# OpenDriveLab/ThinkTwice

Measured on AMD Instinct MI355X. Metric: frames/sec forward (4-cam+LiDAR, thinktwice.py cfg), higher is better.
Workload: dtype bf16x3h; 1 GPU; forward_inference thinktwice.py cfg: 8 frames x (2 sweeps x 4 cams x 448x896 + 65536-pt LiDAR), ResNet50+PAFPN+DepthNet+UNet+LSS splat, LidarNet, fusion, 5-stage decoder; parallelism=replicas x1 (no data-path collective), launch=eager launches, 3 batches in flight on alternating streams, batches_in_flight=3

## Files before the change

### thinktwice_amd/csrc/lidar.hip

```cpp
#include <hipcub/hipcub.hpp>

#include "tt_common.h"

namespace tt {

constexpr unsigned long long kInvalidKey = ~0ull;

struct Dims3 { int z, y, x; };

__global__ void lidar_keys_kernel(const float* __restrict__ pts, int B, int Np, int nfeat, float x0, float y0,
                                  float z0, float vx, float vy, float vz, int gx, int gy, int gz, int zlimit,
                                  unsigned long long* __restrict__ keys, unsigned* __restrict__ vals) {
#pragma clang fp contract(off)
    const long long i = (long long)blockIdx.x * blockDim.x + threadIdx.x;
    if (i >= (long long)B * Np) return;
    const int b = (int)(i / Np);
    const float* p = pts + i * nfeat;
    const int cx = (int)floorf((p[0] - x0) / vx);
    const int cy = (int)floorf((p[1] - y0) / vy);
    const int cz = (int)floorf((p[2] - z0) / vz);
    const bool ok = cx >= 0 && cx < gx && cy >= 0 && cy < gy && cz >= 0 && cz < gz && cz < zlimit;
    keys[i] = ok ? ((((unsigned long long)b * gz + cz) * gy + cy) * gx + cx) : kInvalidKey;
    vals[i] = (unsigned)i;
}

__global__ void mark_heads_kernel(const unsigned long long* __restrict__ keys, long long n, int* __restrict__ flags,
                                  int* __restrict__ n_valid) {
    const long long i = (long long)blockIdx.x * blockDim.x + threadIdx.x;
    if (i >= n) return;
    const unsigned long long k = keys[i];
    const bool valid = k != kInvalidKey;
    flags[i] = (valid && (i == 0 || keys[i - 1] != k)) ? 1 : 0;
    if (valid && (i == n - 1 || keys[i + 1] == kInvalidKey)) *n_valid = (int)(i + 1);
}

__global__ void voxel_heads_kernel(const unsigned long long* __restrict__ keys, const int* __restrict__ flags,
                                   const int* __restrict__ scan, long long n, int gx, int gy, int gz,
                                   int* __restrict__ coords, int* __restrict__ first, int* __restrict__ num_voxels) {
    const long long i = (long long)blockIdx.x * blockDim.x + threadIdx.x;
    if (i >= n) return;
    if (flags[i]) {
        const int v = scan[i];
        unsigned long long k = keys[i];
        const int x = (int)(k % gx); k /= gx;
        const int y = (int)(k % gy); k /= gy;
        const int z = (int)(k % gz); k /= gz;
        coords[v * 4 + 0] = (int)k;
        coords[v * 4 + 1] = z;
        coords[v * 4 + 2] = y;
        coords[v * 4 + 3] = x;
        first[v] = (int)i;
    }
    if (i == n - 1) *num_voxels = scan[i] + flags[i];
}

__global__ void vfe_mean_kernel(const float* __restrict__ pts, const unsigned* __restrict__ vals,
                                const int* __restrict__ first, const int* __restrict__ num_voxels,
                                const int* __restrict__ n_valid, int nfeat, int max_points, long long max_rows,
                                float* __restrict__ feats) {
    const long long t = (long long)blockIdx.x * blockDim.x + threadIdx.x;
    const long long v = t / nfeat;
    const int f = (int)(t % nfeat);
    const int M = *num_voxels;
    if (v >= M || v >= max_rows) return;
    const int s = first[v];
    const int e = (v + 1 < M) ? first[v + 1] : *n_valid;
    const int cnt = min(e - s, max_points);
    float sum = 0.f;
    for (int j = 0; j < cnt; ++j) sum += pts[(long long)vals[s + j] * nfeat + f];
    feats[v * nfeat + f] = sum / (float)cnt;
}


__global__ void cap_head_points_kernel(const unsigned long long* __restrict__ keys, const int* __restrict__ flags,
                                       const int* __restrict__ scan_h, const unsigned* __restrict__ vals, long long n,
                                       int* __restrict__ head_pos, int* __restrict__ pt_flag, int* __restrict__ n_heads) {
    const long long i = (long long)blockIdx.x * blockDim.x + threadIdx.x;
    if (i >= n) return;
    if (flags[i]) {
        head_pos[scan_h[i]] = (int)i;
        pt_flag[vals[i]] = 1;
    }
    if (i == n - 1) *n_heads = scan_h[i] + flags[i];
}

__global__ void cap_keep_kernel(const unsigned long long* __restrict__ keys, const int* __restrict__ flags,
                                const unsigned* __restrict__ vals, const int* __restrict__ scan_p, long long n, int Np, int gx,
                                int gy, int gz, int zlimit, int max_voxels, int* __restrict__ keep) {
    const long long i = (long long)blockIdx.x * blockDim.x + threadIdx.x;
    if (i >= n) return;
    int k = 0;
    if (flags[i]) {
        unsigned long long key = keys[i];
        key /= gx; key /= gy;
        const int z = (int)(key % gz);
        const long long p = vals[i];
        const long long b = p / Np;
        const int rank = scan_p[p] - scan_p[b * Np];
        k = (rank < max_voxels && z < zlimit) ? 1 : 0;
    }
    keep[i] = k;
}

__global__ void cap_emit_kernel(const unsigned long long* __restrict__ keys, const int* __restrict__ keep,
                                const int* __restrict__ scan_k, const int* __restrict__ scan_h,
                                const int* __restrict__ head_pos, const int* __restrict__ n_heads,
                                const int* __restrict__ n_valid, long long n, int gx, int gy, int gz, int* __restrict__ coords,
                                int* __restrict__ first, int* __restrict__ last, int* __restrict__ num_voxels) {
    const long long i = (long long)blockIdx.x * blockDim.x + threadIdx.x;
    if (i >= n) return;
    if (keep[i]) {
        const int v = scan_k[i], h = scan_h[i];
        unsigned long long k = keys[i];
        const int x = (int)(k % gx); k /= gx;
        const int y = (int)(k % gy); k /= gy;
        const int z = (int)(k % gz); k /= gz;
        coords[v * 4 + 0] = (int)k;
        coords[v * 4 + 1] = z;
        coords[v * 4 + 2] = y;
        coords[v * 4 + 3] = x;
        first[v] = (int)i;
        last[v] = (h + 1 < *n_heads) ? head_pos[h + 1] : *n_valid;
    }
    if (i == n - 1) *num_voxels = scan_k[i] + keep[i];
}

__global__ void vfe_mean_capped_kernel(const float* __restrict__ pts, const unsigned* __restrict__ vals,
                                       const int* __restrict__ first, const int* __restrict__ last,
                                       const int* __restrict__ num_voxels, int nfeat, int max_points, long long max_rows,
                                       float* __restrict__ feats) {
    const long long t = (long long)blockIdx.x * blockDim.x + threadIdx.x;
    const long long v = t / nfeat;
    const int f = (int)(t % nfeat);
    if (v >= *num_voxels || v >= max_rows) return;
    const int s = first[v];
    const int cnt = min(last[v] - s, max_points);
    float sum = 0.f;
    for (int j = 0; j < cnt; ++j) sum += pts[(long long)vals[s + j] * nfeat + f];
    feats[v * nfeat + f] = sum / (float)cnt;
}

struct ConvGeom { int kz, ky, kx, sz, sy, sx, pz, py, px; };

__device__ __forceinline__ long long lin_cell(int b, int z, int y, int x, Dims3 d) {
    return (((long long)b * d.z + z) * d.y + y) * d.x + x;
}

__global__ void volume_scatter_kernel(const int* __restrict__ coords, const int* __restrict__ num_rows,
                                      long long max_rows, Dims3 d, int* __restrict__ vol) {
    const long long i = (long long)blockIdx.x * blockDim.x + threadIdx.x;
    if (i >= *num_rows || i >= max_rows) return;
    vol[lin_cell(coords[i * 4], coords[i * 4 + 1], coords[i * 4 + 2], coords[i * 4 + 3], d)] = (int)i;
}

__global__ void mark_outputs_kernel(const int* __restrict__ in_coords, const int* __restrict__ in_rows,
                                    long long max_in, ConvGeom g, Dims3 od, int* __restrict__ flags) {
    const int KV = g.kz * g.ky * g.kx;
    const long long t = (long long)blockIdx.x * blockDim.x + threadIdx.x;
    const long long i = t / KV;
    const int k = (int)(t % KV);
    if (i >= *in_rows || i >= max_in) return;
    const int kz = k / (g.ky * g.kx), ky = (k / g.kx) % g.ky, kx = k % g.kx;
    const int nz = in_coords[i * 4 + 1] + g.pz - kz;
    const int ny = in_coords[i * 4 + 2] + g.py - ky;
    const int nx = in_coords[i * 4 + 3] + g.px - kx;
    if (nz < 0 || ny < 0 || nx < 0 || nz % g.sz || ny % g.sy || nx % g.sx) return;
    const int oz = nz / g.sz, oy = ny / g.sy, ox = nx / g.sx;
    if (oz >= od.z || oy >= od.y || ox >= od.x) return;
    flags[lin_cell(in_coords[i * 4], oz, oy, ox, od)] = 1;
}

__global__ void compact_outputs_kernel(const int* __restrict__ flags, const int* __restrict__ scan, long long cells,
                                       Dims3 od, long long max_out, int* __restrict__ vol,
                                       int* __restrict__ out_coords, int* __restrict__ out_rows) {
    const long long c = (long long)blockIdx.x * blockDim.x + threadIdx.x;
    if (c >= cells) return;
    const int f = flags[c];
    const int row = scan[c];
    int v = -1;
    if (f && row < max_out) {
        v = row;
        long long r = c;
        const int x = (int)(r % od.x); r /= od.x;
        const int y = (int)(r % od.y); r /= od.y;
        const int z = (int)(r % od.z); r /= od.z;
        out_coords[(long long)row * 4 + 0] = (int)r;
        out_coords[(long long)row * 4 + 1] = z;
        out_coords[(long long)row * 4 + 2] = y;
        out_coords[(long long)row * 4 + 3] = x;
    }
    vol[c] = v;
    if (c == cells - 1) {
        const long long n = (long long)row + f;
        *out_rows = (int)(n < max_out ? n : max_out);
    }
}

__global__ void rulebook_kernel(const int* __restrict__ out_coords, const int* __restrict__ out_rows, long long max_out,
                                ConvGeom g, Dims3 id, const int* __restrict__ vol, int* __restrict__ nbr) {
    const int KV = g.kz * g.ky * g.kx;
    const long long t = (long long)blockIdx.x * blockDim.x + threadIdx.x;
    const long long o = t / KV;
    const int k = (int)(t % KV);
    if (o >= *out_rows || o >= max_out) return;
    const int kz = k / (g.ky * g.kx), ky = (k / g.kx) % g.ky, kx = k % g.kx;
    const int z = out_coords[o * 4 + 1] * g.sz - g.pz + kz;
    const int y = out_coords[o * 4 + 2] * g.sy - g.py + ky;
    const int x = out_coords[o * 4 + 3] * g.sx - g.px + kx;
    int r = -1;
    if (z >= 0 && z < id.z && y >= 0 && y < id.y && x >= 0 && x < id.x)
        r = vol[lin_cell(out_coords[o * 4], z, y, x, id)];
    nbr[o * KV + k] = r;
}

__global__ void sp_row_masks_kernel(const int* __restrict__ nbr, const int* __restrict__ rows_n, long long max_rows, int KV,
                                    unsigned* __restrict__ keys, unsigned* __restrict__ vals,
                                    unsigned long long* __restrict__ pairs) {
    const long long o = (long long)blockIdx.x * blockDim.x + threadIdx.x;
    unsigned cnt = 0;
    if (o < max_rows) {
        unsigned m = 0xFFFFFFFFu;
        if (o < *rows_n) {
            m = 0;
            for (int t = 0; t < KV; ++t) m |= (nbr[o * KV + t] >= 0 ? 1u : 0u) << t;
            cnt = __popc(m);
        }
        keys[o] = m;
        vals[o] = (unsigned)o;
    }
    if (pairs) {
#pragma unroll
        for (int off = 32; off > 0; off >>= 1) cnt += __shfl_xor(cnt, off);
        if ((threadIdx.x & 63) == 0 && cnt) atomicAdd(pairs, (unsigned long long)cnt);
    }
}

template <typename T>
__global__ void sp_to_dense_kernel(const T* __restrict__ f, const int* __restrict__ coords,
                                   const int* __restrict__ rows_n, long long max_rows, int C, Dims3 d,
                                   T* __restrict__ dense) {
    const long long t = (long long)blockIdx.x * blockDim.x + threadIdx.x;
    const long long r = t / C;
    const int c = (int)(t % C);
    if (r >= *rows_n || r >= max_rows) return;
    const int b = coords[r * 4], z = coords[r * 4 + 1], y = coords[r * 4 + 2], x = coords[r * 4 + 3];
    dense[(((long long)b * d.y + y) * d.x + x) * ((long long)C * d.z) + (long long)c * d.z + z] = f[r * C + c];
}

}

using namespace tt;

static size_t align256(size_t v) { return (v + 255) / 256 * 256; }

extern "C" long long tt_lidar_voxelize_workspace_bytes(long long num_points_total) {
    size_t sort_bytes = 0, scan_bytes = 0;
    const int n = (int)num_points_total;
    (void)hipcub::DeviceRadixSort::SortPairs(nullptr, sort_bytes, (unsigned long long*)nullptr,
                                       (unsigned long long*)nullptr, (unsigned*)nullptr, (unsigned*)nullptr, n);
    (void)hipcub::DeviceScan::ExclusiveSum(nullptr, scan_bytes, (int*)nullptr, (int*)nullptr, n);
    size_t tot = 0;
    tot += 2 * align256(sizeof(unsigned long long) * n);
    tot += 2 * align256(sizeof(unsigned) * n);
    tot += 2 * align256(sizeof(int) * n);
    tot += align256(sizeof(int) * (n + 1));
    tot += align256(sizeof(int) * 4);
    tot += align256(sort_bytes > scan_bytes ? sort_bytes : scan_bytes);
    return (long long)tot;
}

extern "C" int tt_lidar_voxelize(const float* points, int B, int Np, int nfeat, const float* pc_range_lo,
                                 const float* voxel_size, const int* grid_xyz, int z_limit, int max_points,
                                 void* workspace, long long workspace_bytes, float* voxel_feats, int* coords,
                                 int* num_voxels, void* stream) {
    TT_REQUIRE(points && pc_range_lo && voxel_size && grid_xyz && workspace && voxel_feats && coords && num_voxels,
               "tt_lidar_voxelize: null");
    const long long n = (long long)B * Np;
    TT_REQUIRE(n > 0 && n < (1ll << 30), "tt_lidar_voxelize: bad point count");
    TT_REQUIRE(workspace_bytes >= tt_lidar_voxelize_workspace_bytes(n), "tt_lidar_voxelize: workspace too small");
    hipStream_t st = (hipStream_t)stream;
    char* w = (char*)workspace;
    auto take = [&](size_t bytes) { char* p = w; w += align256(bytes); return p; };
    auto* keys_in = (unsigned long long*)take(sizeof(unsigned long long) * n);
    auto* keys_out = (unsigned long long*)take(sizeof(unsigned long long) * n);
    auto* vals_in = (unsigned*)take(sizeof(unsigned) * n);
    auto* vals_out = (unsigned*)take(sizeof(unsigned) * n);
    auto* flags = (int*)take(sizeof(int) * n);
    auto* scan = (int*)take(sizeof(int) * n);
    auto* first = (int*)take(sizeof(int) * (n + 1));
    auto* n_valid = (int*)take(sizeof(int) * 4);
    void* tmp = w;
    size_t tmp_bytes = (size_t)(workspace_bytes - (w - (char*)workspace));
    (void)hipMemsetAsync(n_valid, 0, sizeof(int), st);
    (void)hipMemsetAsync(num_voxels, 0, sizeof(int), st);
    const unsigned blocks = (unsigned)div_up(n, 256);
    hipLaunchKernelGGL(lidar_keys_kernel, dim3(blocks), dim3(256), 0, st, points, B, Np, nfeat, pc_range_lo[0],
                       pc_range_lo[1], pc_range_lo[2], voxel_size[0], voxel_size[1], voxel_size[2], grid_xyz[0],
                       grid_xyz[1], grid_xyz[2], z_limit, keys_in, vals_in);
    size_t sb = tmp_bytes;
    if (hipcub::DeviceRadixSort::SortPairs(tmp, sb, keys_in, keys_out, vals_in, vals_out, (int)n, 0, 64, st) !=
        hipSuccess) {
        set_error("tt_lidar_voxelize: radix sort failed");
        return -2;
    }
    hipLaunchKernelGGL(mark_heads_kernel, dim3(blocks), dim3(256), 0, st, keys_out, n, flags, n_valid);
    sb = tmp_bytes;
    if (hipcub::DeviceScan::ExclusiveSum(tmp, sb, flags, scan, (int)n, st) != hipSuccess) {
        set_error("tt_lidar_voxelize: scan failed");
        return -2;
    }
    hipLaunchKernelGGL(voxel_heads_kernel, dim3(blocks), dim3(256), 0, st, keys_out, flags, scan, n, grid_xyz[0],
                       grid_xyz[1], grid_xyz[2], coords, first, num_voxels);
    hipLaunchKernelGGL(vfe_mean_kernel, dim3((unsigned)div_up(n * nfeat, 256)), dim3(256), 0, st, points, vals_out,
                       first, num_voxels, n_valid, nfeat, max_points, n, voxel_feats);
    return check_launch("tt_lidar_voxelize");
}


extern "C" long long tt_lidar_voxelize_capped_workspace_bytes(long long num_points_total) {
    const long long n = num_points_total;
    return tt_lidar_voxelize_workspace_bytes(n) + (long long)(8 * align256(sizeof(int) * (n + 1)));
}

extern "C" int tt_lidar_voxelize_capped(const float* points, int B, int Np, int nfeat, const float* pc_range_lo,
                                        const float* voxel_size, const int* grid_xyz, int z_limit, int max_points,
                                        int max_voxels, void* workspace, long long workspace_bytes, float* voxel_feats,
                                        int* coords, int* num_voxels, void* stream) {
    TT_REQUIRE(points && pc_range_lo && voxel_size && grid_xyz && workspace && voxel_feats && coords && num_voxels,
               "tt_lidar_voxelize_capped: null");
    const long long n = (long long)B * Np;
    TT_REQUIRE(n > 0 && n < (1ll << 30) && max_voxels > 0, "tt_lidar_voxelize_capped: bad sizes");
    TT_REQUIRE(workspace_bytes >= tt_lidar_voxelize_capped_workspace_bytes(n), "tt_lidar_voxelize_capped: workspace too small");
    hipStream_t st = (hipStream_t)stream;
    char* w = (char*)workspace;
    auto take = [&](size_t bytes) { char* p = w; w += align256(bytes); return p; };
    auto* keys_in = (unsigned long long*)take(sizeof(unsigned long long) * n);
    auto* keys_out = (unsigned long long*)take(sizeof(unsigned long long) * n);
    auto* vals_in = (unsigned*)take(sizeof(unsigned) * n);
    auto* vals_out = (unsigned*)take(sizeof(unsigned) * n);
    auto* flags = (int*)take(sizeof(int) * n);
    auto* scan_h = (int*)take(sizeof(int) * n);
    auto* first = (int*)take(sizeof(int) * (n + 1));
    auto* n_valid = (int*)take(sizeof(int) * 4);
    auto* head_pos = (int*)take(sizeof(int) * (n + 1));
    auto* pt_flag = (int*)take(sizeof(int) * (n + 1));
    auto* scan_p = (int*)take(sizeof(int) * (n + 1));
    auto* keep = (int*)take(sizeof(int) * (n + 1));
    auto* scan_k = (int*)take(sizeof(int) * (n + 1));
    auto* last = (int*)take(sizeof(int) * (n + 1));
    auto* n_heads = (int*)take(sizeof(int) * (n + 1));
    void* tmp = w;
    size_t tmp_bytes = (size_t)(workspace_bytes - (w - (char*)workspace));
    (void)hipMemsetAsync(n_valid, 0, sizeof(int), st);
    (void)hipMemsetAsync(num_voxels, 0, sizeof(int), st);
    (void)hipMemsetAsync(n_heads, 0, sizeof(int), st);
    (void)hipMemsetAsync(pt_flag, 0, sizeof(int) * n, st);
    const unsigned blocks = (unsigned)div_up(n, 256);
    hipLaunchKernelGGL(lidar_keys_kernel, dim3(blocks), dim3(256), 0, st, points, B, Np, nfeat, pc_range_lo[0],
                       pc_range_lo[1], pc_range_lo[2], voxel_size[0], voxel_size[1], voxel_size[2], grid_xyz[0],
                       grid_xyz[1], grid_xyz[2], grid_xyz[2], keys_in, vals_in);
    size_t sb = tmp_bytes;
    if (hipcub::DeviceRadixSort::SortPairs(tmp, sb, keys_in, keys_out, vals_in, vals_out, (int)n, 0, 64, st) != hipSuccess) {
        set_error("tt_lidar_voxelize_capped: radix sort failed");
        return -2;
    }
    hipLaunchKernelGGL(mark_heads_kernel, dim3(blocks), dim3(256), 0, st, keys_out, n, flags, n_valid);
    auto scan = [&](const int* in, int* out) {
        size_t b = tmp_bytes;
        return hipcub::DeviceScan::ExclusiveSum(tmp, b, in, out, (int)n, st) == hipSuccess;
    };
    if (!scan(flags, scan_h)) { set_error("tt_lidar_voxelize_capped: scan failed"); return -2; }
    hipLaunchKernelGGL(cap_head_points_kernel, dim3(blocks), dim3(256), 0, st, keys_out, flags, scan_h, vals_out, n, head_pos,
                       pt_flag, n_heads);
    if (!scan(pt_flag, scan_p)) { set_error("tt_lidar_voxelize_capped: scan failed"); return -2; }
    hipLaunchKernelGGL(cap_keep_kernel, dim3(blocks), dim3(256), 0, st, keys_out, flags, vals_out, scan_p, n, Np, grid_xyz[0],
                       grid_xyz[1], grid_xyz[2], z_limit, max_voxels, keep);
    if (!scan(keep, scan_k)) { set_error("tt_lidar_voxelize_capped: scan failed"); return -2; }
    hipLaunchKernelGGL(cap_emit_kernel, dim3(blocks), dim3(256), 0, st, keys_out, keep, scan_k, scan_h, head_pos, n_heads,
                       n_valid, n, grid_xyz[0], grid_xyz[1], grid_xyz[2], coords, first, last, num_voxels);
    hipLaunchKernelGGL(vfe_mean_capped_kernel, dim3((unsigned)div_up(n * nfeat, 256)), dim3(256), 0, st, points, vals_out,
                       first, last, num_voxels, nfeat, max_points, n, voxel_feats);
    return check_launch("tt_lidar_voxelize_capped");
}

static ConvGeom geom_of(const int* g) { return ConvGeom{g[0], g[1], g[2], g[3], g[4], g[5], g[6], g[7], g[8]}; }

extern "C" int tt_sp_volume_build(const int* coords, const int* num_rows, long long max_rows, int batch,
                                  const int* dims_zyx, int* vol, void* stream) {
    TT_REQUIRE(coords && num_rows && dims_zyx && vol, "tt_sp_volume_build: null");
    hipStream_t st = (hipStream_t)stream;
    Dims3 d{dims_zyx[0], dims_zyx[1], dims_zyx[2]};
    const long long cells = (long long)batch * d.z * d.y * d.x;
    (void)hipMemsetAsync(vol, 0xFF, sizeof(int) * cells, st);
    hipLaunchKernelGGL(volume_scatter_kernel, dim3((unsigned)div_up(max_rows, 256)), dim3(256), 0, st, coords,
                       num_rows, max_rows, d, vol);
    return check_launch("tt_sp_volume_build");
}

extern "C" long long tt_sp_strided_outputs_workspace_bytes(long long out_cells) {
    size_t scan_bytes = 0;
    (void)hipcub::DeviceScan::ExclusiveSum(nullptr, scan_bytes, (int*)nullptr, (int*)nullptr, (int)out_cells);
    return (long long)(2 * align256(sizeof(int) * out_cells) + align256(scan_bytes));
}

extern "C" int tt_sp_strided_outputs(const int* in_coords, const int* in_rows, long long max_in, int batch,
                                     const int* kernel_stride_pad, const int* out_dims_zyx, void* workspace,
                                     long long workspace_bytes, int* out_vol, int* out_coords, int* out_rows,
                                     long long max_out, void* stream) {
    TT_REQUIRE(in_coords && in_rows && kernel_stride_pad && out_dims_zyx && workspace && out_vol && out_coords &&
                   out_rows, "tt_sp_strided_outputs: null");
    hipStream_t st = (hipStream_t)stream;
    ConvGeom g = geom_of(kernel_stride_pad);
    Dims3 od{out_dims_zyx[0], out_dims_zyx[1], out_dims_zyx[2]};
    const long long cells = (long long)batch * od.z * od.y * od.x;
    TT_REQUIRE(cells < (1ll << 31), "tt_sp_strided_outputs: grid too large");
    TT_REQUIRE(workspace_bytes >= tt_sp_strided_outputs_workspace_bytes(cells), "tt_sp_strided_outputs: workspace");
    char* w = (char*)workspace;
    int* flags = (int*)w;
    int* scan = (int*)(w + align256(sizeof(int) * cells));
    void* tmp = w + 2 * align256(sizeof(int) * cells);
    size_t tmp_bytes = (size_t)(workspace_bytes - 2 * (long long)align256(sizeof(int) * cells));
    (void)hipMemsetAsync(flags, 0, sizeof(int) * cells, st);
    const long long t = max_in * g.kz * g.ky * g.kx;
    hipLaunchKernelGGL(mark_outputs_kernel, dim3((unsigned)div_up(t, 256)), dim3(256), 0, st, in_coords, in_rows,
                       max_in, g, od, flags);
    if (hipcub::DeviceScan::ExclusiveSum(tmp, tmp_bytes, flags, scan, (int)cells, st) != hipSuccess) {
        set_error("tt_sp_strided_outputs: scan failed");
        return -2;
    }
    hipLaunchKernelGGL(compact_outputs_kernel, dim3((unsigned)div_up(cells, 256)), dim3(256), 0, st, flags, scan,
                       cells, od, max_out, out_vol, out_coords, out_rows);
    return check_launch("tt_sp_strided_outputs");
}

extern "C" int tt_sp_rulebook(const int* out_coords, const int* out_rows, long long max_out,
                              const int* kernel_stride_pad, const int* in_dims_zyx, const int* in_vol, int* nbr,
                              void* stream) {
    TT_REQUIRE(out_coords && out_rows && kernel_stride_pad && in_dims_zyx && in_vol && nbr, "tt_sp_rulebook: null");
    ConvGeom g = geom_of(kernel_stride_pad);
    Dims3 id{in_dims_zyx[0], in_dims_zyx[1], in_dims_zyx[2]};
    const long long t = max_out * g.kz * g.ky * g.kx;
    hipLaunchKernelGGL(rulebook_kernel, dim3((unsigned)div_up(t, 256)), dim3(256), 0, (hipStream_t)stream, out_coords,
                       out_rows, max_out, g, id, in_vol, nbr);
    return check_launch("tt_sp_rulebook");
}

extern "C" int tt_sp_to_dense(const void* feats, const int* coords, const int* num_rows, long long max_rows, int C,
                              const int* dims_zyx, void* dense, int dtype, void* stream) {
    TT_REQUIRE(feats && coords && num_rows && dims_zyx && dense, "tt_sp_to_dense: null");
    Dims3 d{dims_zyx[0], dims_zyx[1], dims_zyx[2]};
    const dim3 grid((unsigned)div_up(max_rows * C, 256));
    if (dtype == TT_F32)
        hipLaunchKernelGGL(sp_to_dense_kernel<float>, grid, dim3(256), 0, (hipStream_t)stream, (const float*)feats,
                           coords, num_rows, max_rows, C, d, (float*)dense);
    else
        hipLaunchKernelGGL(sp_to_dense_kernel<uint16_t>, grid, dim3(256), 0, (hipStream_t)stream,
                           (const uint16_t*)feats, coords, num_rows, max_rows, C, d, (uint16_t*)dense);
    return check_launch("tt_sp_to_dense");
}

extern "C" long long tt_sp_tile_plan_workspace_bytes(long long max_rows) {
    size_t sort_bytes = 0;
    (void)hipcub::DeviceRadixSort::SortPairs(nullptr, sort_bytes, (unsigned*)nullptr, (unsigned*)nullptr, (unsigned*)nullptr,
                                       (unsigned*)nullptr, (int)max_rows);
    return (long long)(2 * align256(sizeof(unsigned) * max_rows) + align256(sort_bytes));
}

extern "C" int tt_sp_tile_plan(const int* nbr, const int* num_rows, long long max_rows, int KV, void* workspace,
                               long long workspace_bytes, int* row_perm, unsigned* row_mask_sorted,
                               unsigned long long* pairs_or_null, void* stream) {
    TT_REQUIRE(nbr && num_rows && workspace && row_perm && row_mask_sorted, "tt_sp_tile_plan: null");
    TT_REQUIRE(KV >= 1 && KV <= 31 && max_rows > 0 && max_rows < (1ll << 31), "tt_sp_tile_plan: KV=%d max_rows=%lld", KV,
               max_rows);
    TT_REQUIRE(workspace_bytes >= tt_sp_tile_plan_workspace_bytes(max_rows), "tt_sp_tile_plan: workspace too small");
    hipStream_t st = (hipStream_t)stream;
    char* w = (char*)workspace;
    unsigned* keys = (unsigned*)w;
    unsigned* vals = (unsigned*)(w + align256(sizeof(unsigned) * max_rows));
    void* tmp = w + 2 * align256(sizeof(unsigned) * max_rows);
    size_t tmp_bytes = (size_t)(workspace_bytes - 2 * (long long)align256(sizeof(unsigned) * max_rows));
    hipLaunchKernelGGL(sp_row_masks_kernel, dim3((unsigned)div_up(max_rows, 256)), dim3(256), 0, st, nbr, num_rows, max_rows,
                       KV, keys, vals, pairs_or_null);
    if (hipcub::DeviceRadixSort::SortPairs(tmp, tmp_bytes, keys, row_mask_sorted, vals, (unsigned*)row_perm, (int)max_rows, 0,
                                           32, st) != hipSuccess) {
        set_error("tt_sp_tile_plan: radix sort failed");
        return -2;
    }
    return check_launch("tt_sp_tile_plan");
}
```

### thinktwice_amd/csrc/sp_conv_l2.hip

```cpp
#include "conv_lds_dma.h"

namespace tt {

namespace {
constexpr int kL2Taps = 27;
constexpr int kL2Waves = 8;
constexpr int kL2Slab = 32 * (32 + 4) * 4;
}

template <int CIN>
__global__ __launch_bounds__(kL2Waves * 64, 1) void sp_conv_runs_l2_kernel(const ConvArgs p, const float* __restrict__ zp) {
#if defined(__HIP_DEVICE_COMPILE__)
    constexpr int KS = CIN / 16;
    constexpr int ROWB = CIN * 4;
    constexpr int WB = kL2Taps * 32 * ROWB;
    constexpr int NP = WB / 1024;
    constexpr int RPP = 1024 / ROWB, CPR = ROWB / 16;
    static_assert(CIN == 16 || CIN == 32, "one or two k-steps");
    static_assert(WB % 1024 == 0, "whole DMA pieces");

    extern __shared__ __attribute__((aligned(16))) unsigned char smem[];
    const int tid = threadIdx.x, lane = tid & 63, wave = tid >> 6;
    const int wave_s = __builtin_amdgcn_readfirstlane(wave);
    const int n0 = (int)blockIdx.y * 32;
    int Mlim = p.M;
    if (p.m_dev) {
        const int md = *p.m_dev;
        Mlim = md < Mlim ? md : Mlim;
    }
    const int ngroups = (Mlim + 31) >> 5;
    int first = (int)blockIdx.x * kL2Waves;
    const int end = ngroups, stride = (int)gridDim.x * kL2Waves;
    if (first >= end) return;
    first += wave_s;

    const float* __restrict__ in = reinterpret_cast<const float*>(p.in) + p.in_coff;
    const float* __restrict__ wgt = reinterpret_cast<const float*>(p.weight);

    {
        const unsigned lds_base = (unsigned)(uintptr_t)(__attribute__((address_space(3))) unsigned char*)smem;
        const int d_row = lane / CPR, d_pos = lane % CPR;
        for (int i = wave_s; i < NP; i += kL2Waves) {
            const int r = i * RPP + d_row;
            const int t = r >> 5, n = r & 31;
            const int nn = n0 + n < p.Cout ? n0 + n : p.Cout - 1;
            dma_piece(wgt + (long long)nn * p.K + t * CIN + ((d_pos ^ swz<ROWB>(n)) << 2), lds_base + (unsigned)i * 1024u);
        }
    }
    __builtin_amdgcn_s_waitcnt(0x0F70);
    __syncthreads();

    float* const sC = reinterpret_cast<float*>(smem + WB + wave * kL2Slab);
    const unsigned kb = lane >> 5;
    unsigned boff[KS];
#pragma unroll
    for (int ks = 0; ks < KS; ++ks) boff[ks] = frag_off<ROWB>(lane & 31, 4u * ks + kb);
    constexpr unsigned LO = 32u;

    auto load_ent = [&](int g, int (&e)[kL2Taps]) {
        const int m = g * 32 + (lane & 31);
        const bool live = g < end && m < Mlim;
        const int* __restrict__ rb = p.gather + (long long)(live ? m : Mlim - 1) * kL2Taps;
#pragma unroll
        for (int t = 0; t < kL2Taps; ++t) e[t] = rb[t];
#pragma unroll
        for (int t = 0; t < kL2Taps; ++t) e[t] = live ? e[t] : -1;
    };
    auto load_a = [&](int ent, float4 (&a)[KS][2]) {
        const float* __restrict__ row = ent >= 0 ? in + (long long)ent * p.in_cstride : zp;
        const float4* __restrict__ s = reinterpret_cast<const float4*>(row) + 2 * kb;
#pragma unroll
        for (int ks = 0; ks < KS; ++ks) {
            a[ks][0] = s[4 * ks];
            a[ks][1] = s[4 * ks + 1];
        }
    };

    int e[kL2Taps];
    load_ent(first, e);
    for (int g = first; g < end; g += stride) {
        f32x16 acc[1][1];
        zero_acc(acc);
        float4 a[3][KS][2];
        load_a(e[0], a[0]);
        load_a(e[1], a[1]);
        int en[kL2Taps];
        load_ent(g + stride, en);
#pragma unroll
        for (int t = 0; t < kL2Taps; ++t) {
            if (t + 2 < kL2Taps) load_a(e[t + 2], a[(t + 2) % 3]);
            if (__builtin_amdgcn_ballot_w64(e[t] >= 0) == 0ull) continue;
            const unsigned char* wt = smem + t * (32 * ROWB);
#pragma unroll
            for (int ks = 0; ks < KS; ++ks) {
                const uint4 bh = *reinterpret_cast<const uint4*>(wt + boff[ks]);
                const uint4 bl = *reinterpret_cast<const uint4*>(wt + (boff[ks] ^ LO));
                const float4 r0 = a[t % 3][ks][0], r1 = a[t % 3][ks][1];
                const float x[8] = {r0.x, r0.y, r0.z, r0.w, r1.x, r1.y, r1.z, r1.w};
                uint32_t h[4], l[4];
#pragma unroll
                for (int q = 0; q < 4; ++q) {
                    h[q] = pack_bf16x2(x[2 * q], x[2 * q + 1]);
                    const float q0 = x[2 * q] - __uint_as_float(h[q] << 16);
                    const float q1 = x[2 * q + 1] - __uint_as_float(h[q] & 0xffff0000u);
                    l[q] = pack_bf16x2(q0, q1);
                }
                const uint4 ah = uint4{h[0], h[1], h[2], h[3]}, al = uint4{l[0], l[1], l[2], l[3]};
                Mfma<uint16_t>::run(al, bh, acc[0][0]);
                Mfma<uint16_t>::run(ah, bl, acc[0][0]);
                Mfma<uint16_t>::run(ah, bh, acc[0][0]);
            }
        }
        if (p.act != 99)
            conv_epilogue_vec<float, 4, 1, 1, 32, 32, true>(p, acc, sC, lane, 0, 0, g * 32, n0, Mlim);
#pragma unroll
        for (int t = 0; t < kL2Taps; ++t) e[t] = en[t];
    }
#endif
}

template <int CIN>
static int launch_l2(ConvArgs& a, hipStream_t st) {
    constexpr size_t smem = (size_t)kL2Taps * 32 * CIN * 4 + (size_t)kL2Waves * kL2Slab;
    static_assert(smem <= 160 * 1024, "the CU's LDS");
    auto kern = sp_conv_runs_l2_kernel<CIN>;
    const void* zp = zero_page("sp_conv_runs_l2_kernel");
    if (!zp || lds_opt_in(reinterpret_cast<const void*>(kern), smem, "sp_conv_runs_l2_kernel")) return -1;
    const int ncol = div_up(a.Cout, 32);
    int gx = div_up(a.M, kL2Waves * 32);
    if (gx > kNumCU / ncol) gx = kNumCU / ncol;
    a.tiles_n = ncol;
    a.splits = 1;
    a.ws = nullptr;
    a.m_begin = 0;
    hipLaunchKernelGGL(kern, dim3((unsigned)gx, (unsigned)ncol), dim3(kL2Waves * 64), smem, st, a, reinterpret_cast<const float*>(zp));
    return 1;
}

int launch_sp_conv_l2(const ConvChoice& c, ConvArgs& a, hipStream_t st) {
    if (a.Cin == 32 && c.bkb == 128) return launch_l2<32>(a, st);
    if (a.Cin == 16 && c.bkb == 64) return launch_l2<16>(a, st);
    TT_REQUIRE(false, "tt_conv2d_fwd: no sp_conv_runs_l2_kernel for Cin = %d", a.Cin);
}

}
```

Measured before the change: 108.4 frames/s.

## Rewrite sparse conv index kernels: per-row marking, vectorized compaction, 3x3x3 rulebook

Sparse-conv index building changes in three places. Output marking now uses one thread per input row that walks only the stride-compatible taps, and compaction handles four cells per thread with int4 loads and stores. A dedicated 3x3x3 rulebook kernel reads three contiguous x-neighbours per (z,y) line, stages the 27 entries in shared memory and writes them out coalesced. The L2 conv's prefetch ring depth becomes a compile-time macro, left at its old value of 3. These paths add alignment checks and fallbacks, and cast some indices to 32-bit, which narrows the sizes they can handle.

```diff
diff --git a/thinktwice_amd/csrc/lidar.hip b/thinktwice_amd/csrc/lidar.hip
--- a/thinktwice_amd/csrc/lidar.hip
+++ b/thinktwice_amd/csrc/lidar.hip
@@ -153,46 +153,118 @@
     vol[lin_cell(coords[i * 4], coords[i * 4 + 1], coords[i * 4 + 2], coords[i * 4 + 3], d)] = (int)i;
 }
 
-__global__ void mark_outputs_kernel(const int* __restrict__ in_coords, const int* __restrict__ in_rows,
-                                    long long max_in, ConvGeom g, Dims3 od, int* __restrict__ flags) {
-    const int KV = g.kz * g.ky * g.kx;
-    const long long t = (long long)blockIdx.x * blockDim.x + threadIdx.x;
-    const long long i = t / KV;
-    const int k = (int)(t % KV);
-    if (i >= *in_rows || i >= max_in) return;
-    const int kz = k / (g.ky * g.kx), ky = (k / g.kx) % g.ky, kx = k % g.kx;
-    const int nz = in_coords[i * 4 + 1] + g.pz - kz;
-    const int ny = in_coords[i * 4 + 2] + g.py - ky;
-    const int nx = in_coords[i * 4 + 3] + g.px - kx;
-    if (nz < 0 || ny < 0 || nx < 0 || nz % g.sz || ny % g.sy || nx % g.sx) return;
-    const int oz = nz / g.sz, oy = ny / g.sy, ox = nx / g.sx;
-    if (oz >= od.z || oy >= od.y || ox >= od.x) return;
-    flags[lin_cell(in_coords[i * 4], oz, oy, ox, od)] = 1;
-}
-
-__global__ void compact_outputs_kernel(const int* __restrict__ flags, const int* __restrict__ scan, long long cells,
-                                       Dims3 od, long long max_out, int* __restrict__ vol,
-                                       int* __restrict__ out_coords, int* __restrict__ out_rows) {
-    const long long c = (long long)blockIdx.x * blockDim.x + threadIdx.x;
-    if (c >= cells) return;
-    const int f = flags[c];
-    const int row = scan[c];
-    int v = -1;
-    if (f && row < max_out) {
-        v = row;
-        long long r = c;
-        const int x = (int)(r % od.x); r /= od.x;
-        const int y = (int)(r % od.y); r /= od.y;
-        const int z = (int)(r % od.z); r /= od.z;
-        out_coords[(long long)row * 4 + 0] = (int)r;
-        out_coords[(long long)row * 4 + 1] = z;
-        out_coords[(long long)row * 4 + 2] = y;
-        out_coords[(long long)row * 4 + 3] = x;
-    }
-    vol[c] = v;
-    if (c == cells - 1) {
-        const long long n = (long long)row + f;
-        *out_rows = (int)(n < max_out ? n : max_out);
+constexpr int kSpIdxRows = 256;
+constexpr int kSpIdxMaxBlocks = 1024;
+
+__global__ __launch_bounds__(kSpIdxRows) void mark_outputs_kernel(const int4* __restrict__ in_coords,
+                                                                  const int* __restrict__ in_rows, long long max_in, ConvGeom g,
+                                                                  Dims3 od, int* __restrict__ flags) {
+    const long long n = min((long long)*in_rows, max_in);
+    for (long long i = (long long)blockIdx.x * kSpIdxRows + threadIdx.x; i < n; i += (long long)gridDim.x * kSpIdxRows) {
+        const int4 c = in_coords[i];
+        const int az = c.y + g.pz, ay = c.z + g.py, ax = c.w + g.px;
+        const int qz = az / g.sz, qy = ay / g.sy, qx = ax / g.sx;
+        const int rz = az - qz * g.sz, ry = ay - qy * g.sy, rx = ax - qx * g.sx;
+        for (int kz = rz, oz = qz; kz < g.kz && oz >= 0; kz += g.sz, --oz) {
+            if (oz >= od.z) continue;
+            for (int ky = ry, oy = qy; ky < g.ky && oy >= 0; ky += g.sy, --oy) {
+                if (oy >= od.y) continue;
+                int* __restrict__ line = flags + ((c.x * od.z + oz) * od.y + oy) * od.x;
+                for (int kx = rx, ox = qx; kx < g.kx && ox >= 0; kx += g.sx, --ox)
+                    if (ox < od.x) line[ox] = 1;
+            }
+        }
+    }
+}
+
+template <int V>
+__global__ __launch_bounds__(256) void compact_outputs_kernel(const int* __restrict__ flags, const int* __restrict__ scan,
+                                                              int cells, Dims3 od, int max_out, int* __restrict__ vol,
+                                                              int* __restrict__ out_coords, int* __restrict__ out_rows) {
+    const int t = (int)blockIdx.x * 256 + (int)threadIdx.x;
+    const int quads = V == 4 ? cells >> 2 : 0;
+    auto cell = [&](int c, int f, int row) -> int {
+        if (c == cells - 1) {
+            const int n = row + f;
+            *out_rows = n < max_out ? n : max_out;
+        }
+        if (!f || row >= max_out) return -1;
+        unsigned r = (unsigned)c;
+        const unsigned yq = r / (unsigned)od.x, x = r - yq * (unsigned)od.x;
+        const unsigned zq = yq / (unsigned)od.y, y = yq - zq * (unsigned)od.y;
+        const unsigned b = zq / (unsigned)od.z, z = zq - b * (unsigned)od.z;
+        if (V == 4) {
+            reinterpret_cast<int4*>(out_coords)[row] = int4{(int)b, (int)z, (int)y, (int)x};
+        } else {
+            out_coords[row * 4ll + 0] = (int)b;
+            out_coords[row * 4ll + 1] = (int)z;
+            out_coords[row * 4ll + 2] = (int)y;
+            out_coords[row * 4ll + 3] = (int)x;
+        }
+        return row;
+    };
+    if (t < quads) {
+        const int4 f = reinterpret_cast<const int4*>(flags)[t], s = reinterpret_cast<const int4*>(scan)[t];
+        int4 v;
+        v.x = cell(4 * t, f.x, s.x);
+        v.y = cell(4 * t + 1, f.y, s.y);
+        v.z = cell(4 * t + 2, f.z, s.z);
+        v.w = cell(4 * t + 3, f.w, s.w);
+        reinterpret_cast<int4*>(vol)[t] = v;
+    } else {
+        const int c = 4 * quads + (t - quads);
+        if (c < cells) vol[c] = cell(c, flags[c], scan[c]);
+    }
+}
+
+typedef int i32x4 __attribute__((ext_vector_type(4)));
+
+__global__ __launch_bounds__(kSpIdxRows) void rulebook27_kernel(const int4* __restrict__ out_coords,
+                                                                const int* __restrict__ out_rows, int max_out, ConvGeom g,
+                                                                Dims3 id, const int* __restrict__ vol, int* __restrict__ nbr) {
+    __shared__ __attribute__((aligned(16))) int s_nbr[kSpIdxRows * 27];
+    const int n = min(*out_rows, max_out);
+    const int tid = (int)threadIdx.x;
+    const long long sample = (long long)id.z * id.y * id.x;
+    for (int row0 = (int)blockIdx.x * kSpIdxRows; row0 < n; row0 += (int)gridDim.x * kSpIdxRows) {
+        const int cnt = min(kSpIdxRows, n - row0);
+        if (tid < cnt) {
+            const int4 c = out_coords[row0 + tid];
+            const int* __restrict__ vb = vol + c.x * sample;
+            const int z0 = c.y * g.sz - g.pz, y0 = c.z * g.sy - g.py, x0 = c.w * g.sx - g.px;
+            const int xa = min(max(x0, 0), id.x - 3);
+            int v[9][3];
+#pragma unroll
+            for (int l = 0; l < 9; ++l) {
+                const int z = min(max(z0 + l / 3, 0), id.z - 1), y = min(max(y0 + l % 3, 0), id.y - 1);
+                const int* __restrict__ line = vb + (z * id.y + y) * id.x + xa;
+                v[l][0] = line[0];
+                v[l][1] = line[1];
+                v[l][2] = line[2];
+            }
+            int* __restrict__ s = s_nbr + tid * 27;
+            const int d = x0 - xa;
+            const bool in0 = x0 >= 0 && x0 < id.x, in1 = x0 + 1 >= 0 && x0 + 1 < id.x, in2 = x0 + 2 >= 0 && x0 + 2 < id.x;
+#pragma unroll
+            for (int l = 0; l < 9; ++l) {
+                const int z = z0 + l / 3, y = y0 + l % 3;
+                const bool ok = z >= 0 && z < id.z && y >= 0 && y < id.y;
+                const int a = v[l][0], b = v[l][1], c2 = v[l][2];
+                const int o0 = d == 0 ? a : d == 1 ? b : d == 2 ? c2 : -1;
+                const int o1 = d == 0 ? b : d == 1 ? c2 : d == -1 ? a : -1;
+                const int o2 = d == 0 ? c2 : d == -1 ? b : d == -2 ? a : -1;
+                s[l * 3 + 0] = ok && in0 ? o0 : -1;
+                s[l * 3 + 1] = ok && in1 ? o1 : -1;
+                s[l * 3 + 2] = ok && in2 ? o2 : -1;
+            }
+        }
+        __syncthreads();
+        const int total = cnt * 27, quads = total >> 2;
+        int* __restrict__ dst = nbr + row0 * 27;
+        for (int i = tid; i < quads; i += kSpIdxRows)
+            reinterpret_cast<i32x4*>(dst)[i] = reinterpret_cast<const i32x4*>(s_nbr)[i];
+        if (4 * quads + tid < total) dst[4 * quads + tid] = s_nbr[4 * quads + tid];
+        __syncthreads();
     }
 }
 
@@ -385,6 +457,13 @@
 
 static ConvGeom geom_of(const int* g) { return ConvGeom{g[0], g[1], g[2], g[3], g[4], g[5], g[6], g[7], g[8]}; }
 
+static bool aligned16(const void* p) { return ((uintptr_t)p & 15u) == 0; }
+
+static int idx_blocks(long long max_rows) {
+    const long long b = (max_rows + kSpIdxRows - 1) / kSpIdxRows;
+    return (int)(b < kSpIdxMaxBlocks ? b : kSpIdxMaxBlocks);
+}
+
 extern "C" int tt_sp_volume_build(const int* coords, const int* num_rows, long long max_rows, int batch,
                                   const int* dims_zyx, int* vol, void* stream) {
     TT_REQUIRE(coords && num_rows && dims_zyx && vol, "tt_sp_volume_build: null");
@@ -420,16 +499,23 @@
     int* scan = (int*)(w + align256(sizeof(int) * cells));
     void* tmp = w + 2 * align256(sizeof(int) * cells);
     size_t tmp_bytes = (size_t)(workspace_bytes - 2 * (long long)align256(sizeof(int) * cells));
+    TT_REQUIRE(max_in > 0 && max_out > 0 && g.sz > 0 && g.sy > 0 && g.sx > 0 && g.pz >= 0 && g.py >= 0 && g.px >= 0,
+               "tt_sp_strided_outputs: bad geometry");
+    TT_REQUIRE(aligned16(in_coords), "tt_sp_strided_outputs: in_coords must be 16-byte aligned");
     (void)hipMemsetAsync(flags, 0, sizeof(int) * cells, st);
-    const long long t = max_in * g.kz * g.ky * g.kx;
-    hipLaunchKernelGGL(mark_outputs_kernel, dim3((unsigned)div_up(t, 256)), dim3(256), 0, st, in_coords, in_rows,
-                       max_in, g, od, flags);
+    hipLaunchKernelGGL(mark_outputs_kernel, dim3((unsigned)idx_blocks(max_in)), dim3(kSpIdxRows), 0, st,
+                       reinterpret_cast<const int4*>(in_coords), in_rows, max_in, g, od, flags);
     if (hipcub::DeviceScan::ExclusiveSum(tmp, tmp_bytes, flags, scan, (int)cells, st) != hipSuccess) {
         set_error("tt_sp_strided_outputs: scan failed");
         return -2;
     }
-    hipLaunchKernelGGL(compact_outputs_kernel, dim3((unsigned)div_up(cells, 256)), dim3(256), 0, st, flags, scan,
-                       cells, od, max_out, out_vol, out_coords, out_rows);
+    const int mo = (int)(max_out < cells ? max_out : cells);
+    if (aligned16(out_vol) && aligned16(out_coords) && aligned16(workspace))
+        hipLaunchKernelGGL(compact_outputs_kernel<4>, dim3((unsigned)div_up(cells / 4 + cells % 4, 256)), dim3(256), 0, st,
+                           flags, scan, (int)cells, od, mo, out_vol, out_coords, out_rows);
+    else
+        hipLaunchKernelGGL(compact_outputs_kernel<1>, dim3((unsigned)div_up(cells, 256)), dim3(256), 0, st, flags, scan,
+                           (int)cells, od, mo, out_vol, out_coords, out_rows);
     return check_launch("tt_sp_strided_outputs");
 }
 
@@ -439,8 +525,14 @@
     TT_REQUIRE(out_coords && out_rows && kernel_stride_pad && in_dims_zyx && in_vol && nbr, "tt_sp_rulebook: null");
     ConvGeom g = geom_of(kernel_stride_pad);
     Dims3 id{in_dims_zyx[0], in_dims_zyx[1], in_dims_zyx[2]};
+    if (g.kz == 3 && g.ky == 3 && g.kx == 3 && id.x >= 3 && id.z > 0 && id.y > 0 && max_out > 0 && max_out * 27 < (1ll << 31) &&
+        (long long)id.z * id.y * id.x < (1ll << 31) && aligned16(out_coords) && aligned16(nbr)) {
+        hipLaunchKernelGGL(rulebook27_kernel, dim3((unsigned)idx_blocks(max_out)), dim3(kSpIdxRows), 0, (hipStream_t)stream,
+                           reinterpret_cast<const int4*>(out_coords), out_rows, (int)max_out, g, id, in_vol, nbr);
+        return check_launch("tt_sp_rulebook");
+    }
     const long long t = max_out * g.kz * g.ky * g.kx;
-    hipLaunchKernelGGL(rulebook_kernel, dim3((unsigned)div_up(t, 256)), dim3(256), 0, (hipStream_t)stream, out_coords,
+    hipLaunchKernelGGL(rulebook_kernel,dim3((unsigned)div_up(t, 256)), dim3(256), 0, (hipStream_t)stream, out_coords,
                        out_rows, max_out, g, id, in_vol, nbr);
     return check_launch("tt_sp_rulebook");
 }
diff --git a/thinktwice_amd/csrc/sp_conv_l2.hip b/thinktwice_amd/csrc/sp_conv_l2.hip
--- a/thinktwice_amd/csrc/sp_conv_l2.hip
+++ b/thinktwice_amd/csrc/sp_conv_l2.hip
@@ -6,6 +6,11 @@
 constexpr int kL2Taps = 27;
 constexpr int kL2Waves = 8;
 constexpr int kL2Slab = 32 * (32 + 4) * 4;
+#ifndef TT_SP_L2_RING
+#define TT_SP_L2_RING 3
+#endif
+constexpr int kL2Ring = TT_SP_L2_RING;
+static_assert(kL2Ring >= 2 && kL2Ring <= kL2Taps, "ring");
 }
 
 template <int CIN>
@@ -81,21 +86,21 @@
     for (int g = first; g < end; g += stride) {
         f32x16 acc[1][1];
         zero_acc(acc);
-        float4 a[3][KS][2];
-        load_a(e[0], a[0]);
-        load_a(e[1], a[1]);
+        float4 a[kL2Ring][KS][2];
+#pragma unroll
+        for (int t = 0; t < kL2Ring - 1; ++t) load_a(e[t], a[t]);
         int en[kL2Taps];
         load_ent(g + stride, en);
 #pragma unroll
         for (int t = 0; t < kL2Taps; ++t) {
-            if (t + 2 < kL2Taps) load_a(e[t + 2], a[(t + 2) % 3]);
+            if (t + kL2Ring - 1 < kL2Taps) load_a(e[t + kL2Ring - 1], a[(t + kL2Ring - 1) % kL2Ring]);
             if (__builtin_amdgcn_ballot_w64(e[t] >= 0) == 0ull) continue;
             const unsigned char* wt = smem + t * (32 * ROWB);
 #pragma unroll
             for (int ks = 0; ks < KS; ++ks) {
                 const uint4 bh = *reinterpret_cast<const uint4*>(wt + boff[ks]);
                 const uint4 bl = *reinterpret_cast<const uint4*>(wt + (boff[ks] ^ LO));
-                const float4 r0 = a[t % 3][ks][0], r1 = a[t % 3][ks][1];
+                const float4 r0 = a[t % kL2Ring][ks][0], r1 = a[t % kL2Ring][ks][1];
                 const float x[8] = {r0.x, r0.y, r0.z, r0.w, r1.x, r1.y, r1.z, r1.w};
                 uint32_t h[4], l[4];
 #pragma unroll
```

Result: no change. 109.4 frames/s (median of 6 runs) (+0.9%).
